# rom1504/clip-retrieval

Measured on AMD Instinct MI355X. Metric: images/sec embedded (ViT-L/14 bs=256; each sample = image + caption through both towers), higher is better.
Workload: dtype bf16

## Files before the change

### clip-retrieval_amd/csrc/clip_kernels.hip

```cpp

#include <hip/hip_runtime.h>
#include <stdint.h>
#include <stdlib.h>
#include <math.h>
#include "clip_kernels.h"
#include "gemm_common.h"
#include "clipx_attn_plan.h"

namespace clipx {

constexpr int G_TM = 128, G_TN = 128, G_BK = 64;
constexpr int G_STAGE_BYTES = (G_TM + G_TN) * G_BK * 2;
constexpr int G_GROUP_M = 8;

template <int EPI, bool GLDS, bool DEEP = false, bool F16 = false>
__global__ __launch_bounds__(256, (DEEP && !CLIPX_MFMA16) ? 1 : 2) void gemm_bf16_kernel(const bf16* __restrict__ A, const bf16* __restrict__ W,
                                                          const float* __restrict__ bias, void* __restrict__ outp,
                                                          const float* __restrict__ table, int T, int M, int N,
                                                          int K, int row0, const float* __restrict__ rowscale,
                                                          bf16* __restrict__ out16, int kz) {
  extern __shared__ __attribute__((aligned(16))) unsigned char smem[];
  const int tid = threadIdx.x;
  const int lane = tid & 63, w = tid >> 6;
  const int wn = w & 1, wm = w >> 1;
// ... 136 lines not shown
  D_DSREAD(Wd[sl][0], fW16[sl] + (so), 0);               \
  D_DSREAD(Wd[sl][1], fW16[sl] + (so), 2048);            \
  D_DSREAD(Wd[sl][2], fW16[sl] + (so), 4096);            \
  D_DSREAD(Wd[sl][3], fW16[sl] + (so), 6144);
#define D_READ_A(u, so)                                                \
  D_DSREAD(Ad[(u) & 1][0], fA16[(u) >> 1] + (so), ((u) & 1) * 2048);     \
  D_DSREAD(Ad[(u) & 1][1], fA16[(u) >> 1] + (so), 4096 + ((u) & 1) * 2048);
#define D_READ_U0(so) D_READ_W(0, so) D_READ_A(0, so) __builtin_amdgcn_sched_barrier(0);
#define D_READ_U1(so) D_READ_A(1, so) __builtin_amdgcn_sched_barrier(0);
#define D_READ_U2(so) D_READ_W(1, so) D_READ_A(2, so) __builtin_amdgcn_sched_barrier(0);
#define D_READ_U3(so) D_READ_A(3, so) __builtin_amdgcn_sched_barrier(0);
#define D_WAIT_N(n) asm volatile("s_waitcnt lgkmcnt(%0)" ::"n"(n) : "memory"); __builtin_amdgcn_sched_barrier(0);
#define D_MFMA_U(u)                                                                                                  \
  _Pragma("unroll") for (int i = 0; i < 2; ++i) _Pragma("unroll") for (int j = 0; j < 2; ++j)                        \
      _Pragma("unroll") for (int j2 = 0; j2 < 2; ++j2)                                                               \
          acc[i][j][2 * ((u) & 1) + j2] =                                                                            \
              mfma_16x16x32<F16>(Wd[(u) >> 1][2 * i + j2], Ad[(u) & 1][j], acc[i][j][2 * ((u) & 1) + j2]);           \
  __builtin_amdgcn_sched_barrier(0);
#else
#define D_READ(F, so, kk)                          \
  D_DSREAD(F[0], fW[kk] + (so), 0);                \
  D_DSREAD(F[1], fW[kk] + (so), 4096);             \
  D_DSREAD(F[2], fA[kk] + (so), 0);                \
  D_DSREAD(F[3], fA[kk] + (so), 4096);             \
  __builtin_amdgcn_sched_barrier(0);
#define D_WAIT_PREV() asm volatile("s_waitcnt lgkmcnt(4)" ::: "memory"); __builtin_amdgcn_sched_barrier(0);
#define D_MFMA(F)                                                                                                   \
  _Pragma("unroll") for (int i = 0; i < 2; ++i) _Pragma("unroll") for (int j = 0; j < 2; ++j) acc[i][j] =            \
      mfma_32x32x16<F16>(F[i], F[2 + j], acc[i][j]);                                                                   \
  __builtin_amdgcn_sched_barrier(0);
#endif
#define D_DMA(off, base, dst)                                                                                         \
  asm volatile("s_mov_b32 m0, %2\n\ts_nop 3\n\tglobal_load_lds_dwordx4 %0, %1" ::"v"(off), "s"(base), "s"(dst) : "memory")
      auto stage = [&](int t, int slot) {
        const char* bw = reinterpret_cast<const char*>(W) + (size_t)(t0 + t) * (G_BK * 2);
        const char* ba = reinterpret_cast<const char*>(A) + (size_t)(t0 + t) * (G_BK * 2);
        const unsigned d = lds_base + slot * G_STAGE_BYTES + wu * 4096;
#pragma unroll
        for (int i = 0; i < 4; ++i) {
          D_DMA(offW[i], bw, d + i * 1024);
          D_DMA(offA[i], ba, d + G_TN * G_BK * 2 + i * 1024);
        }
        __builtin_amdgcn_sched_barrier(0);
      };
      const int npro = nk < 4 ? nk : 4;
      for (int t = 0; t < npro; ++t) stage(t, t);
      if (npro == 4) asm volatile("s_waitcnt vmcnt(24)" ::: "memory");
      else if (npro == 3) asm volatile("s_waitcnt vmcnt(16)" ::: "memory");
      else if (npro == 2) asm volatile("s_waitcnt vmcnt(8)" ::: "memory");
      else asm volatile("s_waitcnt vmcnt(0)" ::: "memory");
      __builtin_amdgcn_sched_barrier(0);
      __builtin_amdgcn_s_barrier();
      __builtin_amdgcn_sched_barrier(0);
#if CLIPX_MFMA16
      D_READ_U0(0u)
      unsigned so = 0;
#define D_KT_HEAD()                                   \
  D_READ_U1(so) D_WAIT_N(2) D_MFMA_U(0)                \
  D_READ_U2(so) D_WAIT_N(6) D_MFMA_U(1)                \
  D_READ_U3(so) D_WAIT_N(2) D_MFMA_U(2)                \
  asm volatile("s_waitcnt lgkmcnt(0)" ::: "memory");  \
  __builtin_amdgcn_sched_barrier(0);
#define D_READ_FIRST(so_) D_READ_U0(so_)
#define D_MFMA_LAST() D_MFMA_U(3)
#else
      D_READ(F0, 0u, 0)
      unsigned so = 0;
#define D_KT_HEAD()                                   \
  D_READ(F1, so, 1) D_WAIT_PREV() D_MFMA(F0)           \
  D_READ(F0, so, 2) D_WAIT_PREV() D_MFMA(F1)           \
  D_READ(F1, so, 3) D_WAIT_PREV() D_MFMA(F0)           \
  asm volatile("s_waitcnt lgkmcnt(0)" ::: "memory");  \
  __builtin_amdgcn_sched_barrier(0);
#define D_READ_FIRST(so_) D_READ(F0, so_, 0)
#define D_MFMA_LAST() D_MFMA(F1)
#endif
#define D_SYNC(vm)                                           \
  asm volatile("s_waitcnt vmcnt(%0)" ::"i"(vm) : "memory");  \
  __builtin_amdgcn_sched_barrier(0);                         \
  __builtin_amdgcn_s_barrier();                              \
  __builtin_amdgcn_sched_barrier(0);
      int t = 0;
      for (; t + 4 < nk; ++t) {
        D_KT_HEAD()
        D_SYNC(16)
        stage(t + 4, t & 3);
        so = (so + G_STAGE_BYTES) & (4 * G_STAGE_BYTES - 1);
        D_READ_FIRST(so)
        D_MFMA_LAST()
      }
      for (; t < nk; ++t) {
        const int rem = nk - 1 - t;
        D_KT_HEAD()
        if (rem >= 3) { D_SYNC(16) } else if (rem == 2) { D_SYNC(8) } else { D_SYNC(0) }
        so = (so + G_STAGE_BYTES) & (4 * G_STAGE_BYTES - 1);
        if (rem > 0) { D_READ_FIRST(so) }
        D_MFMA_LAST()
      }
#undef D_DSREAD
#undef D_READ_FIRST
#undef D_MFMA_LAST
#undef D_DMA
#undef D_KT_HEAD
#undef D_SYNC
    } else {
    issue(0, 0);
    asm volatile("s_waitcnt vmcnt(0)" ::: "memory");
    __syncthreads();
    for (int t = 0; t < nk; ++t) {
      if (t + 1 < nk) issue(t + 1, (t + 1) & 1);
      compute(t & 1);
      asm volatile("s_waitcnt vmcnt(0)" ::: "memory");
      __syncthreads();
    }
    }
  } else {
    uint4 rw0, rw1, rw2, rw3, ra0, ra1, ra2, ra3;
#define G_LOAD(t)                                                             \
  {                                                                           \
    rw0 = *reinterpret_cast<const uint4*>(gW[0] + (size_t)(t) * G_BK);        \
    rw1 = *reinterpret_cast<const uint4*>(gW[1] + (size_t)(t) * G_BK);        \
    rw2 = *reinterpret_cast<const uint4*>(gW[2] + (size_t)(t) * G_BK);        \
    rw3 = *reinterpret_cast<const uint4*>(gW[3] + (size_t)(t) * G_BK);        \
    ra0 = *reinterpret_cast<const uint4*>(gA[0] + (size_t)(t) * G_BK);        \
    ra1 = *reinterpret_cast<const uint4*>(gA[1] + (size_t)(t) * G_BK);        \
    ra2 = *reinterpret_cast<const uint4*>(gA[2] + (size_t)(t) * G_BK);        \
    ra3 = *reinterpret_cast<const uint4*>(gA[3] + (size_t)(t) * G_BK);        \
  }
#define G_STORE(buf)                                                                        \
  {                                                                                         \
    unsigned char* dW = smem + (buf) * G_STAGE_BYTES + stage_off + lane * 16;               \
    *reinterpret_cast<uint4*>(dW) = rw0;                                                    \
    *reinterpret_cast<uint4*>(dW + 1024) = rw1;                                             \
    *reinterpret_cast<uint4*>(dW + 2048) = rw2;                                             \
    *reinterpret_cast<uint4*>(dW + 3072) = rw3;                                             \
    *reinterpret_cast<uint4*>(dW + G_TN * G_BK * 2) = ra0;                                  \
    *reinterpret_cast<uint4*>(dW + G_TN * G_BK * 2 + 1024) = ra1;                           \
    *reinterpret_cast<uint4*>(dW + G_TN * G_BK * 2 + 2048) = ra2;                           \
    *reinterpret_cast<uint4*>(dW + G_TN * G_BK * 2 + 3072) = ra3;                           \
  }
    G_LOAD(0)
    G_STORE(0)
    __syncthreads();
    for (int t = 0; t < nk; ++t) {
      if (t + 1 < nk) G_LOAD(t + 1)
      compute(t & 1);
      if (t + 1 < nk) G_STORE((t + 1) & 1)
      __syncthreads();
    }
#undef G_LOAD
#undef G_STORE
  }

#pragma unroll
  for (int j = 0; j < 2; ++j) {
#pragma unroll
    for (int i = 0; i < 2; ++i) {
#pragma unroll
      for (int g = 0; g < 4; ++g) {
        const int m = m0 + wm * 64 + j * 32 + quad_m(g, lane);
        if (m >= M) continue;
        const int n = n0 + wn * 64 + i * 32 + quad_n(g, lane);
        const float4 v = make_float4(G_ACC(i, j, g, 0), G_ACC(i, j, g, 1), G_ACC(i, j, g, 2), G_ACC(i, j, g, 3));
        gemm_store_quad<EPI>(v, m, n, N, bias, outp, table, T, row0, rowscale, out16);
      }
    }
  }
}

template <int EPI, bool F16 = false>
static hipError_t launch_gemm_epi(const GemmArgs& g, hipStream_t st) {
  const int ntm = (g.M + G_TM - 1) / G_TM, ntn = g.N / G_TN;
  const dim3 grid(ntm * ntn), block(256);
  const size_t smem = 2 * G_STAGE_BYTES;
  const bool small_off = (size_t)g.M * g.K * 2 < ((size_t)1 << 32) && (size_t)g.N * g.K * 2 < ((size_t)1 << 32);
  if (g.variant == 1 && g.K >= 2 * G_BK && small_off) {
    auto kern = gemm_bf16_kernel<EPI, true, true, F16>;
    const size_t smem4 = 4 * G_STAGE_BYTES;
    hipError_t e = hipFuncSetAttribute(reinterpret_cast<const void*>(kern), hipFuncAttributeMaxDynamicSharedMemorySize, (int)smem4);
    if (e != hipSuccess) return e;
    launch_with_events(g.events, kern, grid, block, smem4, st, g.A, g.W, g.bias, g.out, g.table, g.T, g.M, g.N, g.K, g.row0, g.rowscale, g.out16, 0);
  } else if (g.variant == 1) {
    auto kern = gemm_bf16_kernel<EPI, true, false, F16>;
    hipError_t e = hipFuncSetAttribute(reinterpret_cast<const void*>(kern), hipFuncAttributeMaxDynamicSharedMemorySize, (int)smem);
    if (e != hipSuccess) return e;
    launch_with_events(g.events, kern, grid, block, smem, st, g.A, g.W, g.bias, g.out, g.table, g.T, g.M, g.N, g.K, g.row0, g.rowscale, g.out16, 0);
  } else {
    auto kern = gemm_bf16_kernel<EPI, false, false, F16>;
    hipError_t e = hipFuncSetAttribute(reinterpret_cast<const void*>(kern), hipFuncAttributeMaxDynamicSharedMemorySize, (int)smem);
    if (e != hipSuccess) return e;
    launch_with_events(g.events, kern, grid, block, smem, st, g.A, g.W, g.bias, g.out, g.table, g.T, g.M, g.N, g.K, g.row0, g.rowscale, g.out16, 0);
  }
  return hipGetLastError();
}

template <int EPI>
__global__ __launch_bounds__(256) void splitk_reduce_kernel(const float* __restrict__ part, int S, int M, int N,
                                                           const float* __restrict__ bias, void* __restrict__ outp,
                                                           const float* __restrict__ rowscale, bf16* __restrict__ out16) {
  const int64_t q = (int64_t)blockIdx.x * 256 + threadIdx.x;
  const int nq4 = N >> 2;
  if (q >= (int64_t)M * nq4) return;
  const int m = (int)(q / nq4), n = (int)(q - (int64_t)m * nq4) * 4;
  float4 v = *reinterpret_cast<const float4*>(part + (size_t)m * N + n);
  for (int z = 1; z < S; ++z) {
    const float4 p = *reinterpret_cast<const float4*>(part + ((size_t)z * M + m) * N + n);
    v.x += p.x; v.y += p.y; v.z += p.z; v.w += p.w;
  }
  gemm_store_quad<EPI>(v, m, n, N, bias, outp, nullptr, 1, 0, rowscale, out16);
}

static int splitk_factor(const GemmArgs& g) {
  if (!g.splitk_ws || g.M > 1024 || g.epi == EPI_TABLE_F32 || g.epi == EPI_RAW_F32) return 1;
  const int nk = g.K / G_BK;
  if (nk < 8 || (nk < 32 && g.M > G_TM)) return 1;
  const int cu = g.n_cu > 0 ? g.n_cu : 256;
  const int tiles = ((g.M + G_TM - 1) / G_TM) * (g.N / G_TN);
  int S = 1;
  for (int c = 2; c <= 16; ++c) {
    if (nk % c != 0 || nk / c < 4) continue;
    if ((size_t)c * g.M * g.N * sizeof(float) > g.splitk_ws_bytes) break;
    if (tiles * (c - 1) >= cu) break;
    S = c;
  }
  return S;
}

template <int EPI>
static hipError_t launch_splitk_epi(const GemmArgs& g, int S, hipStream_t st) {
  const int ntm = (g.M + G_TM - 1) / G_TM, ntn = g.N / G_TN;
  auto kern = g.f16 ? gemm_bf16_kernel<EPI_RAW_F32, true, true, true> : gemm_bf16_kernel<EPI_RAW_F32, true, true, false>;
  const size_t smem4 = 4 * G_STAGE_BYTES;
  hipError_t e = hipFuncSetAttribute(reinterpret_cast<const void*>(kern), hipFuncAttributeMaxDynamicSharedMemorySize, (int)smem4);
  if (e != hipSuccess) return e;
  launch_with_events(g.events, kern, dim3(ntm * ntn, S), dim3(256), smem4, st, g.A, g.W, nullptr, g.splitk_ws, nullptr, 1, g.M, g.N, g.K, 0,
                     nullptr, nullptr, (g.K / G_BK) / S);
  const int64_t quads = (int64_t)g.M * (g.N / 4);
  launch_with_events(g.events, splitk_reduce_kernel<EPI>, dim3((unsigned)((quads + 255) / 256)), dim3(256), 0, st, g.splitk_ws, S, g.M, g.N,
                     g.bias, g.out, g.rowscale, g.out16);
  return hipGetLastError();
}

static hipError_t launch_gemm128(const GemmArgs& g, hipStream_t st) {
  const bool small_off = (size_t)g.M * g.K * 2 < ((size_t)1 << 32) && (size_t)g.N * g.K * 2 < ((size_t)1 << 32);
  const int S = (g.variant == 1 && small_off) ? splitk_factor(g) : 1;
  if (S > 1) {
    switch (g.epi) {
      case EPI_BIAS_BF16: return launch_splitk_epi<EPI_BIAS_BF16>(g, S, st);
      case EPI_BIAS_F16: return launch_splitk_epi<EPI_BIAS_F16>(g, S, st);
      case EPI_BIAS_QGELU_BF16: return launch_splitk_epi<EPI_BIAS_QGELU_BF16>(g, S, st);
      case EPI_BIAS_GELU_BF16: return launch_splitk_epi<EPI_BIAS_GELU_BF16>(g, S, st);
      case EPI_BIAS_RESID_F32: return launch_splitk_epi<EPI_BIAS_RESID_F32>(g, S, st);
      case EPI_BIAS_RESID_H16: return launch_splitk_epi<EPI_BIAS_RESID_H16>(g, S, st);
      default: break;
    }
  }
  if (g.f16) {
    switch (g.epi) {
      case EPI_BIAS_BF16: return launch_gemm_epi<EPI_BIAS_BF16, true>(g, st);
      case EPI_BIAS_F16: return launch_gemm_epi<EPI_BIAS_F16, true>(g, st);
      case EPI_BIAS_QGELU_BF16: return launch_gemm_epi<EPI_BIAS_QGELU_BF16, true>(g, st);
      case EPI_BIAS_GELU_BF16: return launch_gemm_epi<EPI_BIAS_GELU_BF16, true>(g, st);
      default: return hipErrorInvalidValue;
    }
  }
  switch (g.epi) {
    case EPI_BIAS_BF16: return launch_gemm_epi<EPI_BIAS_BF16>(g, st);
    case EPI_BIAS_F16: return launch_gemm_epi<EPI_BIAS_F16>(g, st);
    case EPI_BIAS_QGELU_BF16: return launch_gemm_epi<EPI_BIAS_QGELU_BF16>(g, st);
    case EPI_BIAS_GELU_BF16: return launch_gemm_epi<EPI_BIAS_GELU_BF16>(g, st);
    case EPI_BIAS_RESID_F32: return launch_gemm_epi<EPI_BIAS_RESID_F32>(g, st);
    case EPI_BIAS_RESID_H16: return launch_gemm_epi<EPI_BIAS_RESID_H16>(g, st);
    case EPI_TABLE_F32: return launch_gemm_epi<EPI_TABLE_F32>(g, st);
    default: return hipErrorInvalidValue;
  }
}

int gemm256_bulk_mtiles(int M, int N, int n_cu) {
  const int mt = M / 256, nt = N / 256;
  if (mt <= 0 || nt <= 0) return 0;
  const int cu = (n_cu > 0 ? n_cu : 256) & ~7;
  int best = mt;
  double best_cost = 1e30;
  for (int peel = 0; peel <= 8 && peel < mt; ++peel) {
    const int bulk = mt - peel;
    const int rounds = (bulk * nt + cu - 1) / cu;
    const double rest = (double)(peel * 4 * nt) / (2.0 * cu);
    const double cost = rounds + (peel ? 0.25 * (rest > 1.0 ? rest : 1.0) / 0.6 : 0.0);
    if (cost < best_cost - 1e-9) { best_cost = cost; best = bulk; }
  }
  return best;
}

int gemm256_tail_blocks(int N, int K, int n_cu) {
  int grid = (n_cu > 0 ? n_cu : 256) & ~7;
  if (grid < 8) grid = 8;
  if (N % 32 || K % 128 || (size_t)32 * K * 2 >= ((size_t)1 << 31)) return 0;
  const int cb = N / 32;
  for (int nb = 1; nb <= 4; ++nb)
    if (cb % nb == 0 && 8 * (cb / nb) <= grid) return nb;
  return 0;
}

int gemm256_dispatch_mtiles(int M, int N, int K, int variant, int n_cu) {
  if (variant < 2 || N % 256 != 0 || K % 128 != 0 || M < 256) return 0;
  const int bulk = gemm256_bulk_mtiles(M, N, n_cu);
  const int cu = (n_cu > 0 ? n_cu : 256);
  return bulk > 0 && (int64_t)bulk * (N / 256) >= cu / 2 ? bulk : 0;
}

int gemm256_whole_tile_rows(int M, int N, int K, int variant, int n_cu) {
  const int Mp = (M + 255) / 256 * 256;
  return Mp != M && gemm256_dispatch_mtiles(Mp, N, K, variant, n_cu) > 0 ? Mp : M;
}

hipError_t launch_gemm(const GemmArgs& g0, hipStream_t st) {
  GemmArgs g = g0;
  if (g.M <= 0 || g.N % G_TN != 0 || g.K % G_BK != 0 || g.K <= 0) return hipErrorInvalidValue;
  const bool out16 = g.epi == EPI_BIAS_BF16 || g.epi == EPI_BIAS_QGELU_BF16 || g.epi == EPI_BIAS_GELU_BF16 || g.epi == EPI_BIAS_F16;
  if (out16 && !g.rowscale) return hipErrorInvalidValue;
  if (g.f16 && !out16) return hipErrorInvalidValue;
  if (g.stats_eps > 0.f) {
    if (!g.f16 || !out16) return hipErrorInvalidValue;
    int fused_rows = 0;
    if (g.variant == 6 && g.N % 256 == 0 && g.K % 128 == 0 && g.M >= 256) {
      const int bulk = gemm256_bulk_mtiles(g.M, g.N, g.n_cu);
      const int cu = (g.n_cu > 0 ? g.n_cu : 256);
      GemmArgs b = g;
      b.M = bulk * 256;
      if (bulk > 0 && (int64_t)bulk * (g.N / 256) >= cu / 2 && gemm256w4_fuses_stats(b)) fused_rows = b.M;
    }
    if (fused_rows < g.M) {
      hipError_t e = launch_rowstats(reinterpret_cast<const char*>(g.A) + (size_t)fused_rows * g.K * 2, const_cast<float*>(g.rowscale) + fused_rows,
                                     g.M - fused_rows, g.K, g.stats_eps, st, 1, g.range_flag, 1, g.events);
      if (e != hipSuccess) return e;
    }
    if (fused_rows == 0) g.stats_eps = 0.f;
  }
  {
    const int bulk = gemm256_dispatch_mtiles(g.M, g.N, g.K, g.variant, g.n_cu);
    if (bulk > 0) {
      GemmArgs b = g;
      b.M = bulk * 256;
      b.tail_m0 = b.tail_nb = 0;
      if (g.M - b.M == 256 && (g.variant == 3 || g.variant == 6) && g.row0 == 0) {
        b.tail_nb = gemm256_tail_blocks(g.N, g.K, g.n_cu);
        b.tail_m0 = b.M;
      }
      const bool tail_inside = b.tail_nb > 0;
      hipError_t e = (g.variant == 6 && gemm256w4_supports(b)) ? launch_gemm256w4(b, g.n_cu, st) : launch_gemm256sp(b, g.n_cu, st);
      if (e != hipSuccess) return e;
      if (b.M == g.M || tail_inside) return hipSuccess;
      GemmArgs r = g;
      r.variant = 1;
      r.stats_eps = 0.f;
      r.splitk_ws = nullptr;
      r.A = g.A + (size_t)b.M * g.K;
      r.M = g.M - b.M;
      const size_t esz = (g.epi == EPI_BIAS_RESID_F32 || g.epi == EPI_TABLE_F32) ? 4 : 2;
      r.out = reinterpret_cast<char*>(g.out) + (size_t)b.M * g.N * esz;
      r.row0 = g.row0 + b.M;
      if (g.rowscale) r.rowscale = g.rowscale + b.M;
      if (g.out16) r.out16 = g.out16 + (size_t)b.M * g.N;
      return launch_gemm128(r, st);
    }
  }
  GemmArgs r = g;
  if (r.variant >= 2) r.variant = 1;
  r.stats_eps = 0.f;
  return launch_gemm128(r, st);
}

template <int NV, int OUT>
__global__ __launch_bounds__(256) void layernorm_kernel(const float* __restrict__ x, const float* __restrict__ gamma,
                                                       const float* __restrict__ beta, void* __restrict__ y, int M,
                                                       float eps, bf16* __restrict__ y16) {
  constexpr int d = NV * 256;
  const int lane = threadIdx.x & 63;
  const int row = blockIdx.x * 4 + (threadIdx.x >> 6);
  if (row >= M) return;
  const float4* xr = reinterpret_cast<const float4*>(x + (size_t)row * d);
  float4 v[NV];
  float s = 0.f;
#pragma unroll
  for (int e = 0; e < NV; ++e) {
    v[e] = xr[lane + 64 * e];
    s += (v[e].x + v[e].y) + (v[e].z + v[e].w);
  }
  for (int o = 32; o > 0; o >>= 1) s += __shfl_xor(s, o);
  const float mean = s * (1.f / d);
  float q = 0.f;
#pragma unroll
  for (int e = 0; e < NV; ++e) {
    const float a = v[e].x - mean, b = v[e].y - mean, c = v[e].z - mean, dd = v[e].w - mean;
    q += (a * a + b * b) + (c * c + dd * dd);
  }
  for (int o = 32; o > 0; o >>= 1) q += __shfl_xor(q, o);
  const float rstd = 1.f / sqrtf(q * (1.f / d) + eps);
#pragma unroll
  for (int e = 0; e < NV; ++e) {
    const int c4 = lane + 64 * e;
    const float4 g4 = reinterpret_cast<const float4*>(gamma)[c4];
    const float4 b4 = reinterpret_cast<const float4*>(beta)[c4];
    float4 o;
    o.x = (v[e].x - mean) * rstd * g4.x + b4.x;
    o.y = (v[e].y - mean) * rstd * g4.y + b4.y;
    o.z = (v[e].z - mean) * rstd * g4.z + b4.z;
    o.w = (v[e].w - mean) * rstd * g4.w + b4.w;
    if (OUT == 1) {
      bf16x4 ob;
      ob[0] = (bf16)o.x; ob[1] = (bf16)o.y; ob[2] = (bf16)o.z; ob[3] = (bf16)o.w;
      reinterpret_cast<bf16x4*>(reinterpret_cast<bf16*>(y) + (size_t)row * d)[c4] = ob;
    } else if (OUT == 2) {
      f16x4 oh;
      oh[0] = (_Float16)o.x; oh[1] = (_Float16)o.y; oh[2] = (_Float16)o.z; oh[3] = (_Float16)o.w;
      reinterpret_cast<f16x4*>(reinterpret_cast<_Float16*>(y) + (size_t)row * d)[c4] = oh;
    } else {
      reinterpret_cast<float4*>(reinterpret_cast<float*>(y) + (size_t)row * d)[c4] = o;
      if (y16) {
        bf16x4 ob;
        ob[0] = (bf16)o.x; ob[1] = (bf16)o.y; ob[2] = (bf16)o.z; ob[3] = (bf16)o.w;
        reinterpret_cast<bf16x4*>(y16 + (size_t)row * d)[c4] = ob;
      }
    }
  }
}

template <int NV2, bool F16>
__global__ __launch_bounds__(256) void rowstats_kernel(const void* __restrict__ x16, float* __restrict__ rstd, int M, float eps,
                                                       int* __restrict__ range_flag) {
  constexpr int d = NV2 * 256;
  const int lane = threadIdx.x & 63;
  const int row = blockIdx.x * 4 + (threadIdx.x >> 6);
  if (row >= M) return;
  const uint2* xr = reinterpret_cast<const uint2*>(reinterpret_cast<const uint16_t*>(x16) + (size_t)row * d);
  float v[NV2][4];
  float s = 0.f;
#pragma unroll
  for (int e = 0; e < NV2; ++e) {
    const uint2 raw = xr[lane + 64 * e];
    if (F16) {
      const f16x4 h = __builtin_bit_cast(f16x4, raw);
#pragma unroll
      for (int j = 0; j < 4; ++j) v[e][j] = (float)h[j];
    } else {
      const bf16x4 h = __builtin_bit_cast(bf16x4, raw);
#pragma unroll
      for (int j = 0; j < 4; ++j) v[e][j] = (float)h[j];
    }
    s += (v[e][0] + v[e][1]) + (v[e][2] + v[e][3]);
  }
  for (int o = 32; o > 0; o >>= 1) s += __shfl_xor(s, o);
  if (range_flag && lane == 0 && !(fabsf(s) <= 3.0e38f)) atomicOr(range_flag, 1);
  const float mean = s * (1.f / d);
  float q = 0.f;
#pragma unroll
  for (int e = 0; e < NV2; ++e) {
    const float a = v[e][0] - mean, b = v[e][1] - mean, c = v[e][2] - mean, dd = v[e][3] - mean;
    q += (a * a + b * b) + (c * c + dd * dd);
  }
  for (int o = 32; o > 0; o >>= 1) q += __shfl_xor(q, o);
  if (lane == 0) rstd[row] = 1.f / sqrtf(q * (1.f / d) + eps);
}

template <int NV2>
__global__ __launch_bounds__(256) void rowstats_f16_kernel(const void* __restrict__ x16, float* __restrict__ rstd, int M, float eps,
                                                           int* __restrict__ range_flag) {
  constexpr int d = NV2 * 256, NCH = d / 8;
  const int lane = threadIdx.x & 63, q4 = lane >> 4, r16 = lane & 15;
  const int row = (blockIdx.x * 4 + (threadIdx.x >> 6)) * 16 + r16;
  const uint4* xr = reinterpret_cast<const uint4*>(reinterpret_cast<const uint16_t*>(x16) + (size_t)(row < M ? row : M - 1) * d);
  const unsigned ones2 = __builtin_amdgcn_readfirstlane(0x3c003c00u);
  float s1 = 0.f, s2 = 0.f;
  constexpr int U = 8;
  static_assert((NCH / 4) % U == 0, "row length");
  for (int j0 = 0; j0 < NCH / 4; j0 += U) {
    uint4 c[U];
#pragma unroll
    for (int u = 0; u < U; ++u) c[u] = xr[q4 + 4 * (j0 + u)];
#pragma unroll
    for (int u = 0; u < U; ++u) {
      CLIPX_DOT2_SQ(s2, c[u].x); CLIPX_DOT2_SQ(s2, c[u].y); CLIPX_DOT2_SQ(s2, c[u].z); CLIPX_DOT2_SQ(s2, c[u].w);
      CLIPX_DOT2_SUM(s1, c[u].x, ones2); CLIPX_DOT2_SUM(s1, c[u].y, ones2); CLIPX_DOT2_SUM(s1, c[u].z, ones2); CLIPX_DOT2_SUM(s1, c[u].w, ones2);
    }
  }
  s1 += __shfl_xor(s1, 16);
  s2 += __shfl_xor(s2, 16);
  s1 += __shfl_xor(s1, 32);
  s2 += __shfl_xor(s2, 32);
  if (row >= M || q4 != 0) return;
  if (range_flag && !(fabsf(s1) <= 3.0e38f)) atomicOr(range_flag, 1);
  rstd[row] = ln_rstd_onepass(s1, s2, 1.f / (float)d, eps);
}

hipError_t launch_rowstats(const void* x16, float* rstd, int M, int d, float eps, hipStream_t st, int f16, int* range_flag, int canonical,
                           LaunchEvents* events) {
  if (M <= 0) return hipSuccess;
  if (f16 && canonical) {
    const dim3 grid((M + 63) / 64), block(256);
#define RSH_CASE(NV)                                                                                           \
  case NV * 256:                                                                                               \
    launch_with_events(events, rowstats_f16_kernel<NV>, grid, block, 0, st, x16, rstd, M, eps, range_flag);   \
    break;
    switch (d) {
      RSH_CASE(1) RSH_CASE(2) RSH_CASE(3) RSH_CASE(4) RSH_CASE(5) RSH_CASE(6) RSH_CASE(7) RSH_CASE(8)
      default: return hipErrorInvalidValue;
    }
#undef RSH_CASE
    return hipGetLastError();
  }
  const dim3 grid((M + 3) / 4), block(256);
#define RS_CASE(NV)                                                                                        \
  case NV * 256:                                                                                           \
    if (f16) launch_with_events(events, rowstats_kernel<NV, true>, grid, block, 0, st, x16, rstd, M, eps, range_flag);   \
    else launch_with_events(events, rowstats_kernel<NV, false>, grid, block, 0, st, x16, rstd, M, eps, range_flag);      \
    break;
  switch (d) {
    RS_CASE(1) RS_CASE(2) RS_CASE(3) RS_CASE(4) RS_CASE(5) RS_CASE(6) RS_CASE(7) RS_CASE(8)
    default: return hipErrorInvalidValue;
  }
#undef RS_CASE
  return hipGetLastError();
}

__global__ __launch_bounds__(256) void fold_layernorm_kernel(const float* __restrict__ W, const float* __restrict__ gamma,
                                                            const float* __restrict__ beta, const float* __restrict__ bias,
                                                            bf16* __restrict__ Wf, float* __restrict__ cf, int K, int f16) {
  __shared__ float red[8];
  const int n = blockIdx.x, tid = threadIdx.x;
  const float* w = W + (size_t)n * K;
  float sg = 0.f, sb = 0.f;
  for (int k = tid; k < K; k += 256) {
    sg += w[k] * gamma[k];
    sb += w[k] * beta[k];
  }
  for (int o = 32; o > 0; o >>= 1) { sg += __shfl_xor(sg, o); sb += __shfl_xor(sb, o); }
  if ((tid & 63) == 0) { red[tid >> 6] = sg; red[4 + (tid >> 6)] = sb; }
  __syncthreads();
  const float mean = (red[0] + red[1] + red[2] + red[3]) / (float)K;
  for (int k = tid; k < K; k += 256) {
    const float v = w[k] * gamma[k] - mean;
    if (f16) reinterpret_cast<_Float16*>(Wf)[(size_t)n * K + k] = (_Float16)v;
    else Wf[(size_t)n * K + k] = (bf16)v;
  }
  if (tid == 0) cf[n] = bias[n] + (red[4] + red[5] + red[6] + red[7]);
}
hipError_t launch_fold_layernorm(const float* W, const float* gamma, const float* beta, const float* bias, bf16* Wf, float* cf,
                                 int N, int K, hipStream_t st, int f16) {
  hipLaunchKernelGGL(fold_layernorm_kernel, dim3(N), dim3(256), 0, st, W, gamma, beta, bias, Wf, cf, K, f16);
  return hipGetLastError();
}
__global__ void fill_f32_kernel(float* __restrict__ p, float v, int64_t n) {
  for (int64_t i = (int64_t)blockIdx.x * blockDim.x + threadIdx.x; i < n; i += (int64_t)gridDim.x * blockDim.x) p[i] = v;
}
hipError_t launch_fill_f32(float* p, float v, int64_t n, hipStream_t st) {
  if (n <= 0) return hipSuccess;
  hipLaunchKernelGGL(fill_f32_kernel, dim3(256), dim3(256), 0, st, p, v, n);
  return hipGetLastError();
}

hipError_t launch_layernorm(const float* x, const float* gamma, const float* beta, void* y, int out_kind, int M, int d,
                            float eps, hipStream_t st, bf16* y16) {
  if (M <= 0) return hipSuccess;
  const dim3 grid((M + 3) / 4), block(256);
#define LN_CASE(NV)                                                                                           \
  case NV * 256:                                                                                              \
    if (out_kind == 1) hipLaunchKernelGGL((layernorm_kernel<NV, 1>), grid, block, 0, st, x, gamma, beta, y, M, eps, (bf16*)nullptr); \
    else if (out_kind == 2) hipLaunchKernelGGL((layernorm_kernel<NV, 2>), grid, block, 0, st, x, gamma, beta, y, M, eps, (bf16*)nullptr); \
    else hipLaunchKernelGGL((layernorm_kernel<NV, 0>), grid, block, 0, st, x, gamma, beta, y, M, eps, y16);    \
    break;
  switch (d) {
    LN_CASE(1) LN_CASE(2) LN_CASE(3) LN_CASE(4) LN_CASE(5) LN_CASE(6) LN_CASE(7) LN_CASE(8)
    default: return hipErrorInvalidValue;
  }
#undef LN_CASE
  return hipGetLastError();
}

template <int FMT>
__global__ __launch_bounds__(256) void im2col_kernel(const void* __restrict__ pixels, int B, int S, int P, int Kp,
                                                    float m0, float m1, float m2, float i0, float i1, float i2,
                                                    bf16* __restrict__ out) {
  const int gdim = S / P, T = gdim * gdim + 1, PP = P * P, K = 3 * PP, nch = Kp / 8;
  const int64_t total = (int64_t)B * T * nch;
  for (int64_t idx = (int64_t)blockIdx.x * blockDim.x + threadIdx.x; idx < total; idx += (int64_t)gridDim.x * blockDim.x) {
    const int ch = (int)(idx % nch);
    const int64_t row = idx / nch;
    const int t = (int)(row % T), b = (int)(row / T);
    bf16x8 o;
    const int tp = t > 0 ? t - 1 : 0;
    const int py = tp / gdim, px = tp - py * gdim;
    float raw[8];
    int cc[8];
#pragma unroll
    for (int e = 0; e < 8; ++e) {
      const int k = ch * 8 + e;
      const int kk = k < K ? k : K - 1;
      const int c = kk / PP, rem = kk - c * PP;
      const int iy = rem / P, ix = rem - iy * P;
      const int yy = py * P + iy, xx = px * P + ix;
      cc[e] = c;
      if (FMT == 0) raw[e] = reinterpret_cast<const float*>(pixels)[(((size_t)b * 3 + c) * S + yy) * S + xx];
      else raw[e] = (float)reinterpret_cast<const unsigned char*>(pixels)[(((size_t)b * S + yy) * S + xx) * 3 + c];
    }
#pragma unroll
    for (int e = 0; e < 8; ++e) {
      float v = raw[e];
      if (FMT != 0) {
        const int c = cc[e];
        const float mean = c == 0 ? m0 : (c == 1 ? m1 : m2), sd = c == 0 ? i0 : (c == 1 ? i1 : i2);
        v = __fdiv_rn(__fsub_rn(__fdiv_rn(v, 255.f), mean), sd);
      }
      o[e] = (t > 0 && ch * 8 + e < K) ? (bf16)v : (bf16)0.f;
    }
    *reinterpret_cast<bf16x8*>(out + (size_t)row * Kp + ch * 8) = o;
  }
}

hipError_t launch_im2col(const void* pixels, int fmt, int B, int S, int P, int Kp, const float* mean,
                         const float* stdv, bf16* out, hipStream_t st) {
  if (B <= 0) return hipSuccess;
  const int gdim = S / P, T = gdim * gdim + 1;
  const int64_t total = (int64_t)B * T * (Kp / 8);
  const int blocks = (int)((total + 255) / 256 < 65536 * 4 ? (total + 255) / 256 : 65536 * 4);
  if (fmt == 0)
    hipLaunchKernelGGL(im2col_kernel<0>, dim3(blocks), dim3(256), 0, st, pixels, B, S, P, Kp, 0.f, 0.f, 0.f, 1.f, 1.f, 1.f, out);
  else
    hipLaunchKernelGGL(im2col_kernel<1>, dim3(blocks), dim3(256), 0, st, pixels, B, S, P, Kp, mean[0], mean[1], mean[2],
                       stdv[0], stdv[1], stdv[2], out);
  return hipGetLastError();
}

__device__ __forceinline__ f32x16 attn_mfma(bf16x8 a, bf16x8 b, f32x16 c) {
  return __builtin_amdgcn_mfma_f32_32x32x16_f16(__builtin_bit_cast(f16x8, a), __builtin_bit_cast(f16x8, b), c, 0, 0, 0);
}
__device__ __forceinline__ unsigned attn_pack_p(float p0, float p1) {
  typedef float f32x2_t __attribute__((ext_vector_type(2)));
  typedef _Float16 f16x2_t __attribute__((ext_vector_type(2)));
  return __builtin_bit_cast(unsigned, __builtin_convertvector((f32x2_t){p0, p1}, f16x2_t));
}

__device__ long long g_attn_phase[8192 * 4];
#ifdef CLIPX_ABLATE
__device__ int g_attn_pk_timer = 0;
#endif
template <int DH, int NKB, int NW, int QPW, bool CAUSAL, bool RECOMP, bool TIMER = false, bool RAGGED = false>
__global__ __launch_bounds__(NW * 64, NKB > 9 ? (NW + 3) / 4 : (2 * NW + 3) / 4) void attention_kernel(const bf16* __restrict__ qkv, bf16* __restrict__ out, int Tin,
                                                              int H, float scale_log2e, int dbg, int q_blocks,
                                                              const int* __restrict__ offs, const int* __restrict__ lens) {
  constexpr int TP = NKB * 32;
  constexpr int CH = DH / 8;
  constexpr int KS = DH / 16;
  constexpr int KROW = DH == 64 ? 128 : 176;
  constexpr int DV = (DH + 31) / 32 * 32, NB = DV / 32;
  constexpr int VT_STRIDE = TP * 2 + 8;
  extern __shared__ __attribute__((aligned(16))) unsigned char smem[];
  unsigned char* sK = smem;
  unsigned char* sVt = smem + TP * KROW;
  const int tid = threadIdx.x, lane = tid & 63, w = tid >> 6;
  const int hb = lane >> 5, l31 = lane & 31;
  long long tph[4] = {0, 0, 0, 0};
  long long tst = TIMER ? (long long)__builtin_readcyclecounter() : 0;
#define A_STAMP(i) if (TIMER) { const long long n_ = (long long)__builtin_readcyclecounter(); tph[i] += n_ - tst; tst = n_; }
  const int b = blockIdx.x / H, h = blockIdx.x - b * H;
  const int ld = 3 * H * DH;
  const int T = lens ? lens[b] : Tin;
// ... 1335 lines not shown
```

### clip-retrieval_amd/csrc/gemm256_tail.h

```cpp
#pragma once
#include "gemm_common.h"

namespace clipx {

#ifndef S_FENCE
#define S_FENCE() __builtin_amdgcn_sched_barrier(0)
#endif

template <int EPI, bool F16, int NB, int NW = 8>
__device__ __forceinline__ void gemm256_tail(const bf16* __restrict__ A, const bf16* __restrict__ W, const float* __restrict__ bias,
                                             void* __restrict__ outp, const float* __restrict__ table, int T, int N, int K,
                                             const float* __restrict__ rowscale, bf16* __restrict__ out16, int tail_m0,
                                             unsigned char* smem, unsigned lds_base, int w, int lane) {
  constexpr int NOP = 1 + NB;
  constexpr int SB = NOP * 8192;
  constexpr int R = 131072 / SB;
  const int ncg = (N >> 5) / NB;
  const int strip = blockIdx.x;
  if (strip >= 8 * ncg) return;
  const int rb = strip & 7, cg = strip >> 3;
  const int tm = tail_m0 + rb * 32, tn = cg * NB * 32;
  const int l31 = lane & 31, hb = lane >> 5;
#if CLIPX_MFMA16
  const unsigned voff = (unsigned)(((lane & 15) * K + 8 * (lane >> 4)) * 2);
  const char* baseA = reinterpret_cast<const char*>(A) + (size_t)tm * K * 2;
  const char* baseW = reinterpret_cast<const char*>(W) + (size_t)tn * K * 2;
#define T_PIECE(p) ((size_t)(16 * ((p) & 1)) * K * 2 + ((p) >> 1) * 64)
  (void)l31; (void)hb;
#else
  const unsigned voff = (unsigned)((l31 * K + 8 * hb) * 2);
  const char* baseA = reinterpret_cast<const char*>(A) + (size_t)tm * K * 2;
  const char* baseW = reinterpret_cast<const char*>(W) + (size_t)tn * K * 2;
#define T_PIECE(p) ((size_t)(p) * 32)
#endif
  constexpr int PPW = 8 / NW;
  const int nch = K >> 7;
#define T_DMA(off, base, dst) \
  asm volatile("s_mov_b32 m0, %2\n\ts_nop 3\n\tglobal_load_lds_dwordx4 %0, %1" ::"v"(off), "s"(base), "s"(dst) : "memory")
  auto issue = [&](int c, int slot) {
    const int cc = c < nch ? c : nch - 1;
#pragma unroll
    for (int pp = 0; pp < PPW; ++pp) {
      const int p = w + NW * pp;
      const unsigned dst = lds_base + slot * SB + p * 1024;
      T_DMA(voff, baseA + T_PIECE(p) + (size_t)cc * 256, dst);
#pragma unroll
      for (int o = 0; o < NB; ++o) T_DMA(voff, baseW + T_PIECE(p) + (size_t)o * 64 * K + (size_t)cc * 256, dst + (1 + o) * 8192);
    }
    S_FENCE();
  };
#pragma unroll
  for (int c = 0; c < R - 1; ++c) issue(c, c);
#if CLIPX_MFMA16
  f32x4 acc[4];
#pragma unroll
  for (int g = 0; g < 4; ++g) acc[g] = f32x4{0.f, 0.f, 0.f, 0.f};
#define T_ACC(g, e) acc[g][e]
#else
  f32x16 acc;
#pragma unroll
  for (int r = 0; r < 16; ++r) acc[r] = 0.f;
#define T_ACC(g, e) acc[4 * (g) + (e)]
#endif
  int slot = 0;
  for (int c = 0; c < nch; ++c) {
    asm volatile("s_waitcnt vmcnt(%0)" ::"n"((R - 2) * NOP * PPW) : "memory");
    S_FENCE();
    __builtin_amdgcn_s_barrier();
    S_FENCE();
    issue(c + R - 1, slot == 0 ? R - 1 : slot - 1);
    if (w < NB) {
      const unsigned char* st = smem + slot * SB + lane * 16;
#if CLIPX_MFMA16
#pragma unroll
      for (int sl = 0; sl < 4; ++sl) {
        const frag_t af0 = *reinterpret_cast<const frag_t*>(st + (2 * sl) * 1024);
        const frag_t af1 = *reinterpret_cast<const frag_t*>(st + (2 * sl + 1) * 1024);
        const frag_t wf0 = *reinterpret_cast<const frag_t*>(st + (1 + w) * 8192 + (2 * sl) * 1024);
        const frag_t wf1 = *reinterpret_cast<const frag_t*>(st + (1 + w) * 8192 + (2 * sl + 1) * 1024);
        mfma_block16<F16>(acc, wf0, wf1, af0, af1);
      }
#else
#pragma unroll
      for (int ks = 0; ks < 8; ++ks) {
        const frag_t af = *reinterpret_cast<const frag_t*>(st + ks * 1024);
        const frag_t wf = *reinterpret_cast<const frag_t*>(st + (1 + w) * 8192 + ks * 1024);
        acc = mfma_32x32x16<F16>(wf, af, acc);
      }
#endif
    }
    slot = slot + 1 == R ? 0 : slot + 1;
  }
#undef T_DMA
#undef T_PIECE
  asm volatile("s_waitcnt vmcnt(0)" ::: "memory");
  S_FENCE();
  if (w < NB) {
#pragma unroll
    for (int g = 0; g < 4; ++g) {
      const int m = tm + quad_m(g, lane);
      const int n = tn + w * 32 + quad_n(g, lane);
      const float4 v = make_float4(T_ACC(g, 0), T_ACC(g, 1), T_ACC(g, 2), T_ACC(g, 3));
      gemm_store_quad<EPI>(v, m, n, N, bias, outp, table, T, 0, rowscale, out16);
    }
  }
#undef T_ACC
}


}
```

### clip-retrieval_amd/csrc/gemm_common.h

```cpp
#pragma once
#include <hip/hip_runtime.h>
#include <stdint.h>
#include "clip_kernels.h"

namespace clipx {

typedef __bf16 bf16x8 __attribute__((ext_vector_type(8)));
typedef __bf16 bf16x4 __attribute__((ext_vector_type(4)));
typedef float f32x16 __attribute__((ext_vector_type(16)));
typedef float f32x4 __attribute__((ext_vector_type(4)));
typedef _Float16 f16x8 __attribute__((ext_vector_type(8)));
typedef _Float16 f16x4 __attribute__((ext_vector_type(4)));
typedef int frag_t __attribute__((ext_vector_type(4)));

template <bool F16>
__device__ __forceinline__ f32x16 mfma_32x32x16(frag_t a, frag_t b, f32x16 c) {
  if constexpr (F16) return __builtin_amdgcn_mfma_f32_32x32x16_f16(__builtin_bit_cast(f16x8, a), __builtin_bit_cast(f16x8, b), c, 0, 0, 0);
  else return __builtin_amdgcn_mfma_f32_32x32x16_bf16(__builtin_bit_cast(bf16x8, a), __builtin_bit_cast(bf16x8, b), c, 0, 0, 0);
}
#ifndef CLIPX_MFMA16
#define CLIPX_MFMA16 1
#endif

template <bool F16>
__device__ __forceinline__ f32x4 mfma_16x16x32(frag_t a, frag_t b, f32x4 c) {
  if constexpr (F16) return __builtin_amdgcn_mfma_f32_16x16x32_f16(__builtin_bit_cast(f16x8, a), __builtin_bit_cast(f16x8, b), c, 0, 0, 0);
  else return __builtin_amdgcn_mfma_f32_16x16x32_bf16(__builtin_bit_cast(bf16x8, a), __builtin_bit_cast(bf16x8, b), c, 0, 0, 0);
}
template <bool F16>
__device__ __forceinline__ void mfma_block16(f32x4 (&q)[4], frag_t wf0, frag_t wf1, frag_t af0, frag_t af1) {
  q[0] = mfma_16x16x32<F16>(wf0, af0, q[0]);
  q[1] = mfma_16x16x32<F16>(wf1, af0, q[1]);
  q[2] = mfma_16x16x32<F16>(wf0, af1, q[2]);
  q[3] = mfma_16x16x32<F16>(wf1, af1, q[3]);
}
__device__ __forceinline__ int quad_m(int g, int lane) { return CLIPX_MFMA16 ? 16 * (g >> 1) + (lane & 15) : (lane & 31); }
__device__ __forceinline__ int quad_n(int g, int lane) { return CLIPX_MFMA16 ? 16 * (g & 1) + 4 * (lane >> 4) : 8 * g + 4 * (lane >> 5); }

__device__ __forceinline__ float ln_rstd_onepass(float s1, float s2, float inv_d, float eps) {
  const float mean = s1 * inv_d;
  const float ex2 = s2 * inv_d;
  float var = __builtin_fmaf(-mean, mean, ex2);
  var = var > 0.f ? var : 0.f;
  return 1.f / sqrtf(var + eps);
}
#define CLIPX_DOT2_SQ(acc, w) asm volatile("v_dot2_f32_f16 %0, %1, %1, %0" : "+v"(acc) : "v"(w))
#define CLIPX_DOT2_SUM(acc, w, ones) asm volatile("v_dot2_f32_f16 %0, %1, %2, %0" : "+v"(acc) : "v"(w), "s"(ones))

typedef __attribute__((address_space(3))) void* lds_ptr_t;
typedef const __attribute__((address_space(1))) void* gbl_ptr_t;

__device__ __forceinline__ float quick_gelu(float v) {
  return v * __builtin_amdgcn_rcpf(1.f + __builtin_amdgcn_exp2f(-1.702f * 1.4426950408889634f * v));
}
__device__ __forceinline__ float gelu_erf(float v) {
  const float z = fabsf(v) * 0.70710678118654752f;
  const float t = __builtin_amdgcn_rcpf(__builtin_fmaf(0.3275911f, z, 1.f));
  float p = __builtin_fmaf(1.061405429f, t, -1.453152027f);
  p = __builtin_fmaf(p, t, 1.421413741f);
  p = __builtin_fmaf(p, t, -0.284496736f);
  p = __builtin_fmaf(p, t, 0.254829592f);
  const float e = __builtin_amdgcn_exp2f(-1.4426950408889634f * z * z);
  const float erf_abs = __builtin_fmaf(-p * t, e, 1.f);
  return 0.5f * v + 0.5f * fabsf(v) * erf_abs;
}

template <int EPI>
__device__ __forceinline__ void gemm_store_quad(float4 v, int m, int n, int N, const float* __restrict__ bias,
                                                void* __restrict__ outp, const float* __restrict__ table, int T,
                                                int row0, const float* __restrict__ rowscale, bf16* __restrict__ out16) {
  constexpr bool OUT_BF16 = EPI == EPI_BIAS_BF16 || EPI == EPI_BIAS_QGELU_BF16 || EPI == EPI_BIAS_GELU_BF16 || EPI == EPI_BIAS_F16;
  if (EPI == EPI_RAW_F32) {
    *reinterpret_cast<float4*>(reinterpret_cast<float*>(outp) + (size_t)m * N + n) = v;
    return;
  }
  if (EPI != EPI_TABLE_F32) {
    const float4 b4 = *reinterpret_cast<const float4*>(bias + n);
    if (OUT_BF16) {
      const float r = rowscale[m];
      v.x = __builtin_fmaf(v.x, r, b4.x); v.y = __builtin_fmaf(v.y, r, b4.y);
      v.z = __builtin_fmaf(v.z, r, b4.z); v.w = __builtin_fmaf(v.w, r, b4.w);
    } else {
      v.x += b4.x; v.y += b4.y; v.z += b4.z; v.w += b4.w;
    }
  }
  if (EPI == EPI_BIAS_QGELU_BF16) { v.x = quick_gelu(v.x); v.y = quick_gelu(v.y); v.z = quick_gelu(v.z); v.w = quick_gelu(v.w); }
  if (EPI == EPI_BIAS_GELU_BF16) { v.x = gelu_erf(v.x); v.y = gelu_erf(v.y); v.z = gelu_erf(v.z); v.w = gelu_erf(v.w); }
  if (EPI == EPI_BIAS_F16) {
    asm volatile("" : "+v"(v.x), "+v"(v.y), "+v"(v.z), "+v"(v.w));
    f16x4 o;
    o[0] = (_Float16)v.x; o[1] = (_Float16)v.y; o[2] = (_Float16)v.z; o[3] = (_Float16)v.w;
    *reinterpret_cast<f16x4*>(reinterpret_cast<_Float16*>(outp) + (size_t)m * N + n) = o;
  } else if (OUT_BF16) {
    bf16x4 o;
    o[0] = (bf16)v.x; o[1] = (bf16)v.y; o[2] = (bf16)v.z; o[3] = (bf16)v.w;
    *reinterpret_cast<bf16x4*>(reinterpret_cast<bf16*>(outp) + (size_t)m * N + n) = o;
  } else if (EPI == EPI_BIAS_RESID_F32) {
    float4* p = reinterpret_cast<float4*>(reinterpret_cast<float*>(outp) + (size_t)m * N + n);
    float4 o = *p;
    o.x += v.x; o.y += v.y; o.z += v.z; o.w += v.w;
    *p = o;
    if (out16) {
      bf16x4 h;
      h[0] = (bf16)o.x; h[1] = (bf16)o.y; h[2] = (bf16)o.z; h[3] = (bf16)o.w;
      *reinterpret_cast<bf16x4*>(out16 + (size_t)m * N + n) = h;
    }
  } else if (EPI == EPI_BIAS_RESID_H16) {
    f16x4* p = reinterpret_cast<f16x4*>(reinterpret_cast<_Float16*>(outp) + (size_t)m * N + n);
    const f16x4 x4 = *p;
    f16x4 h;
    h[0] = (_Float16)((float)x4[0] + v.x); h[1] = (_Float16)((float)x4[1] + v.y);
    h[2] = (_Float16)((float)x4[2] + v.z); h[3] = (_Float16)((float)x4[3] + v.w);
    *p = h;
  } else {
    const float4 t4 = *reinterpret_cast<const float4*>(table + (size_t)((m + row0) % T) * N + n);
    v.x += t4.x; v.y += t4.y; v.z += t4.z; v.w += t4.w;
    *reinterpret_cast<float4*>(reinterpret_cast<float*>(outp) + (size_t)m * N + n) = v;
  }
}

hipError_t launch_gemm256sp(const GemmArgs& g, int n_cu, hipStream_t st);
bool gemm256w4_supports(const GemmArgs& g);
bool gemm256w4_fuses_stats(const GemmArgs& g);
hipError_t launch_gemm256w4(const GemmArgs& g, int n_cu, hipStream_t st);

}
```

Measured before the change: 6072.

## Add standalone strip GEMM kernel for small-M and tail rows with swizzled LDS

Adds a standalone strip kernel, reusing the fused tail routine, that handles GEMMs with M≤256 and leftover 256-row tails. Before this, those went to the generic 128-tile kernel. The tail routine gets an XOR-swizzled LDS layout for the MFMA16 path and a 'deal' mode that spreads the MFMA quads over all 4 waves instead of idling the extra waves. It also gates fusing the tail into the bulk kernel on whether the bulk tile count is large enough to hide it. This targets poor occupancy and wave imbalance on small GEMMs such as text-tower or tail launches, at the risk of layout bugs and extra launches.

After: 6125, median of 6. About the same (+0.9%).

```diff
diff --git a/clip-retrieval_amd/csrc/clip_kernels.hip b/clip-retrieval_amd/csrc/clip_kernels.hip
--- a/clip-retrieval_amd/csrc/clip_kernels.hip
+++ b/clip-retrieval_amd/csrc/clip_kernels.hip
@@ -462,11 +462,30 @@
   return 0;
 }
 
+static int gemm256_min_tiles(int n_cu) {
+  const int cu = (n_cu > 0 ? n_cu : 256);
+#ifdef CLIPX_ABLATE
+  if (const char* mt = getenv("CLIPX_GEMM_MIN_TILES")) return atoi(mt);
+#endif
+  return cu / 2;
+}
+
 int gemm256_dispatch_mtiles(int M, int N, int K, int variant, int n_cu) {
   if (variant < 2 || N % 256 != 0 || K % 128 != 0 || M < 256) return 0;
   const int bulk = gemm256_bulk_mtiles(M, N, n_cu);
-  const int cu = (n_cu > 0 ? n_cu : 256);
-  return bulk > 0 && (int64_t)bulk * (N / 256) >= cu / 2 ? bulk : 0;
+  return bulk > 0 && (int64_t)bulk * (N / 256) >= gemm256_min_tiles(n_cu) ? bulk : 0;
+}
+
+static bool gemm256_tail_rides(int64_t ntiles, int N, int nb, int n_cu) {
+  int grid = (n_cu > 0 ? n_cu : 256) & ~7;
+  if (grid < 8) grid = 8;
+  const int cpx = grid >> 3, ncg = (N / 32) / nb;
+  return ntiles >= 7 * cpx + ncg;
+}
+
+static int gemm256_strip_width(const GemmArgs& g) {
+  if ((g.variant != 3 && g.variant != 6) || g.splitk_ws || !gemm256_strips_supports(g)) return 0;
+  return gemm256_tail_blocks(g.N, g.K, g.n_cu);
 }
 
 int gemm256_whole_tile_rows(int M, int N, int K, int variant, int n_cu) {
@@ -488,7 +507,7 @@
       const int cu = (g.n_cu > 0 ? g.n_cu : 256);
       GemmArgs b = g;
       b.M = bulk * 256;
-      if (bulk > 0 && (int64_t)bulk * (g.N / 256) >= cu / 2 && gemm256w4_fuses_stats(b)) fused_rows = b.M;
+      if (bulk > 0 && (int64_t)bulk * (g.N / 256) >= gemm256_min_tiles(cu) && gemm256w4_fuses_stats(b)) fused_rows = b.M;
     }
     if (fused_rows < g.M) {
       hipError_t e = launch_rowstats(reinterpret_cast<const char*>(g.A) + (size_t)fused_rows * g.K * 2, const_cast<float*>(g.rowscale) + fused_rows,
@@ -496,6 +515,10 @@
       if (e != hipSuccess) return e;
     }
     if (fused_rows == 0) g.stats_eps = 0.f;
+  }
+  if (g.M <= 256) {
+    const int nb = gemm256_strip_width(g);
+    if (nb > 0) return launch_gemm256_strips(g, nb, st);
   }
   {
     const int bulk = gemm256_dispatch_mtiles(g.M, g.N, g.K, g.variant, g.n_cu);
@@ -504,24 +527,31 @@
       b.M = bulk * 256;
       b.tail_m0 = b.tail_nb = 0;
       if (g.M - b.M == 256 && (g.variant == 3 || g.variant == 6) && g.row0 == 0) {
-        b.tail_nb = gemm256_tail_blocks(g.N, g.K, g.n_cu);
-        b.tail_m0 = b.M;
+        const int nb = gemm256_tail_blocks(g.N, g.K, g.n_cu);
+        if (nb > 0 && gemm256_tail_rides((int64_t)bulk * (g.N / 256), g.N, nb, g.n_cu)) {
+          b.tail_nb = nb;
+          b.tail_m0 = b.M;
+        }
       }
       const bool tail_inside = b.tail_nb > 0;
       hipError_t e = (g.variant == 6 && gemm256w4_supports(b)) ? launch_gemm256w4(b, g.n_cu, st) : launch_gemm256sp(b, g.n_cu, st);
       if (e != hipSuccess) return e;
       if (b.M == g.M || tail_inside) return hipSuccess;
       GemmArgs r = g;
-      r.variant = 1;
       r.stats_eps = 0.f;
       r.splitk_ws = nullptr;
       r.A = g.A + (size_t)b.M * g.K;
       r.M = g.M - b.M;
       const size_t esz = (g.epi == EPI_BIAS_RESID_F32 || g.epi == EPI_TABLE_F32) ? 4 : 2;
       r.out = reinterpret_cast<char*>(g.out) + (size_t)b.M * g.N * esz;
-      r.row0 = g.row0 + b.M;
       if (g.rowscale) r.rowscale = g.rowscale + b.M;
       if (g.out16) r.out16 = g.out16 + (size_t)b.M * g.N;
+      if (r.M == 256 && g.row0 == 0) {
+        const int nb = gemm256_strip_width(r);
+        if (nb > 0) return launch_gemm256_strips(r, nb, st);
+      }
+      r.variant = 1;
+      r.row0 = g.row0 + b.M;
       return launch_gemm128(r, st);
     }
   }
diff --git a/clip-retrieval_amd/csrc/gemm256_strips.hip b/clip-retrieval_amd/csrc/gemm256_strips.hip
--- /dev/null
+++ b/clip-retrieval_amd/csrc/gemm256_strips.hip
@@ -0,0 +1,71 @@
+
+#include <hip/hip_runtime.h>
+#include <stdint.h>
+#include "gemm_common.h"
+#include "gemm256_tail.h"
+
+namespace clipx {
+
+constexpr int STRIPS_LDS = 131072;
+
+template <int EPI, bool F16, int NB>
+__global__ __launch_bounds__(256) void gemm256_strips_kernel(const bf16* __restrict__ A, const bf16* __restrict__ W, const float* __restrict__ bias,
+                                                             void* __restrict__ outp, int N, int K, const float* __restrict__ rowscale, int nrb) {
+  extern __shared__ __attribute__((aligned(16))) unsigned char smem[];
+  const int lane = threadIdx.x & 63;
+  const int w = __builtin_amdgcn_readfirstlane(threadIdx.x >> 6);
+  const unsigned lds_base = __builtin_amdgcn_readfirstlane((unsigned)(uintptr_t)(__attribute__((address_space(3))) unsigned char*)smem);
+  const int strip = ((int)blockIdx.x / nrb) * 8 + (int)blockIdx.x % nrb;
+  gemm256_tail_strip<EPI, F16, NB, 4>(A, W, bias, outp, nullptr, 1, N, K, rowscale, nullptr, 0, smem, lds_base, w, lane, strip);
+}
+
+template <int EPI, bool F16, int NB>
+static hipError_t launch_strips_nb(const GemmArgs& g, hipStream_t st) {
+  auto kern = gemm256_strips_kernel<EPI, F16, NB>;
+  hipError_t e = hipFuncSetAttribute(reinterpret_cast<const void*>(kern), hipFuncAttributeMaxDynamicSharedMemorySize, STRIPS_LDS);
+  if (e != hipSuccess) return e;
+  const int nrb = g.M / 32, ncg = (g.N / 32) / NB;
+  launch_with_events(g.events, kern, dim3(nrb * ncg), dim3(256), (size_t)STRIPS_LDS, st, g.A, g.W, g.bias, g.out, g.N, g.K, g.rowscale, nrb);
+  return hipGetLastError();
+}
+
+template <int EPI, bool F16>
+static hipError_t launch_strips_epi(const GemmArgs& g, int nb, hipStream_t st) {
+  switch (nb) {
+    case 1: return launch_strips_nb<EPI, F16, 1>(g, st);
+    case 2: return launch_strips_nb<EPI, F16, 2>(g, st);
+    case 3: return launch_strips_nb<EPI, F16, 3>(g, st);
+    case 4: return launch_strips_nb<EPI, F16, 4>(g, st);
+    default: return hipErrorInvalidValue;
+  }
+}
+
+bool gemm256_strips_supports(const GemmArgs& g) {
+  if (g.M <= 0 || g.M > 256 || g.M % 32 != 0 || g.N % 32 != 0 || g.K % 128 != 0 || g.row0 != 0) return false;
+  const bool out16 = g.epi == EPI_BIAS_BF16 || g.epi == EPI_BIAS_F16 || g.epi == EPI_BIAS_QGELU_BF16 || g.epi == EPI_BIAS_GELU_BF16;
+  if (out16) return g.rowscale != nullptr;
+  return !g.f16 && g.epi == EPI_BIAS_RESID_H16;
+}
+
+hipError_t launch_gemm256_strips(const GemmArgs& g, int nb, hipStream_t st) {
+  if (!gemm256_strips_supports(g) || nb < 1 || nb > 4 || (g.N / 32) % nb != 0) return hipErrorInvalidValue;
+  if (g.f16) {
+    switch (g.epi) {
+      case EPI_BIAS_BF16: return launch_strips_epi<EPI_BIAS_BF16, true>(g, nb, st);
+      case EPI_BIAS_F16: return launch_strips_epi<EPI_BIAS_F16, true>(g, nb, st);
+      case EPI_BIAS_QGELU_BF16: return launch_strips_epi<EPI_BIAS_QGELU_BF16, true>(g, nb, st);
+      case EPI_BIAS_GELU_BF16: return launch_strips_epi<EPI_BIAS_GELU_BF16, true>(g, nb, st);
+      default: return hipErrorInvalidValue;
+    }
+  }
+  switch (g.epi) {
+    case EPI_BIAS_BF16: return launch_strips_epi<EPI_BIAS_BF16, false>(g, nb, st);
+    case EPI_BIAS_F16: return launch_strips_epi<EPI_BIAS_F16, false>(g, nb, st);
+    case EPI_BIAS_QGELU_BF16: return launch_strips_epi<EPI_BIAS_QGELU_BF16, false>(g, nb, st);
+    case EPI_BIAS_GELU_BF16: return launch_strips_epi<EPI_BIAS_GELU_BF16, false>(g, nb, st);
+    case EPI_BIAS_RESID_H16: return launch_strips_epi<EPI_BIAS_RESID_H16, false>(g, nb, st);
+    default: return hipErrorInvalidValue;
+  }
+}
+
+}
diff --git a/clip-retrieval_amd/csrc/gemm256_tail.h b/clip-retrieval_amd/csrc/gemm256_tail.h
--- a/clip-retrieval_amd/csrc/gemm256_tail.h
+++ b/clip-retrieval_amd/csrc/gemm256_tail.h
@@ -8,24 +8,30 @@
 #endif
 
 template <int EPI, bool F16, int NB, int NW = 8>
-__device__ __forceinline__ void gemm256_tail(const bf16* __restrict__ A, const bf16* __restrict__ W, const float* __restrict__ bias,
-                                             void* __restrict__ outp, const float* __restrict__ table, int T, int N, int K,
-                                             const float* __restrict__ rowscale, bf16* __restrict__ out16, int tail_m0,
-                                             unsigned char* smem, unsigned lds_base, int w, int lane) {
+__device__ __forceinline__ void gemm256_tail_strip(const bf16* __restrict__ A, const bf16* __restrict__ W, const float* __restrict__ bias,
+                                                   void* __restrict__ outp, const float* __restrict__ table, int T, int N, int K,
+                                                   const float* __restrict__ rowscale, bf16* __restrict__ out16, int tail_m0,
+                                                   unsigned char* smem, unsigned lds_base, int w, int lane, int strip) {
   constexpr int NOP = 1 + NB;
   constexpr int SB = NOP * 8192;
   constexpr int R = 131072 / SB;
+  constexpr bool DEAL = CLIPX_MFMA16 && NW == 4 && NB < 4;
   const int ncg = (N >> 5) / NB;
-  const int strip = blockIdx.x;
   if (strip >= 8 * ncg) return;
   const int rb = strip & 7, cg = strip >> 3;
   const int tm = tail_m0 + rb * 32, tn = cg * NB * 32;
   const int l31 = lane & 31, hb = lane >> 5;
 #if CLIPX_MFMA16
-  const unsigned voff = (unsigned)(((lane & 15) * K + 8 * (lane >> 4)) * 2);
+  const int prow = (w & 3) * 8 + (lane >> 3);
+  const unsigned voff = (unsigned)((prow * K + (((lane & 7) ^ ((prow >> 1) & 7)) << 3)) * 2);
   const char* baseA = reinterpret_cast<const char*>(A) + (size_t)tm * K * 2;
   const char* baseW = reinterpret_cast<const char*>(W) + (size_t)tn * K * 2;
-#define T_PIECE(p) ((size_t)(16 * ((p) & 1)) * K * 2 + ((p) >> 1) * 64)
+#define T_PIECE(p) ((size_t)(((p) >> 2) * 128))
+  unsigned fo[2];
+#pragma unroll
+  for (int s2 = 0; s2 < 2; ++s2) fo[s2] = (unsigned)((lane & 15) * 128 + (((4 * s2 + (lane >> 4)) ^ (((lane & 15) >> 1) & 7)) << 4));
+#define T_SLAB(sl) (fo[(sl) & 1] + ((sl) >> 1) * 4096)
+  constexpr unsigned HALF_B = 2048;
   (void)l31; (void)hb;
 #else
   const unsigned voff = (unsigned)((l31 * K + 8 * hb) * 2);
@@ -56,6 +62,13 @@
 #pragma unroll
   for (int g = 0; g < 4; ++g) acc[g] = f32x4{0.f, 0.f, 0.f, 0.f};
 #define T_ACC(g, e) acc[g][e]
+  unsigned qa[NB], qw[NB];
+#pragma unroll
+  for (int i = 0; i < NB; ++i) {
+    const int q = NB * w + i;
+    qa[i] = (unsigned)(((q & 3) >> 1) * HALF_B);
+    qw[i] = (unsigned)((1 + (q >> 2)) * 8192 + (q & 1) * HALF_B);
+  }
 #else
   f32x16 acc;
 #pragma unroll
@@ -69,22 +82,35 @@
     __builtin_amdgcn_s_barrier();
     S_FENCE();
     issue(c + R - 1, slot == 0 ? R - 1 : slot - 1);
-    if (w < NB) {
-      const unsigned char* st = smem + slot * SB + lane * 16;
+    if (DEAL) {
+#if CLIPX_MFMA16
+      const unsigned char* st = smem + slot * SB;
+#pragma unroll
+      for (int sl = 0; sl < 4; ++sl) {
+#pragma unroll
+        for (int i = 0; i < NB; ++i) {
+          const frag_t af = *reinterpret_cast<const frag_t*>(st + qa[i] + T_SLAB(sl));
+          const frag_t wf = *reinterpret_cast<const frag_t*>(st + qw[i] + T_SLAB(sl));
+          acc[i] = mfma_16x16x32<F16>(wf, af, acc[i]);
+        }
+      }
+#endif
+    } else if (w < NB) {
+      const unsigned char* st = smem + slot * SB;
 #if CLIPX_MFMA16
 #pragma unroll
       for (int sl = 0; sl < 4; ++sl) {
-        const frag_t af0 = *reinterpret_cast<const frag_t*>(st + (2 * sl) * 1024);
-        const frag_t af1 = *reinterpret_cast<const frag_t*>(st + (2 * sl + 1) * 1024);
-        const frag_t wf0 = *reinterpret_cast<const frag_t*>(st + (1 + w) * 8192 + (2 * sl) * 1024);
-        const frag_t wf1 = *reinterpret_cast<const frag_t*>(st + (1 + w) * 8192 + (2 * sl + 1) * 1024);
+        const frag_t af0 = *reinterpret_cast<const frag_t*>(st + T_SLAB(sl));
+        const frag_t af1 = *reinterpret_cast<const frag_t*>(st + T_SLAB(sl) + HALF_B);
+        const frag_t wf0 = *reinterpret_cast<const frag_t*>(st + (1 + w) * 8192 + T_SLAB(sl));
+        const frag_t wf1 = *reinterpret_cast<const frag_t*>(st + (1 + w) * 8192 + T_SLAB(sl) + HALF_B);
         mfma_block16<F16>(acc, wf0, wf1, af0, af1);
       }
 #else
 #pragma unroll
       for (int ks = 0; ks < 8; ++ks) {
-        const frag_t af = *reinterpret_cast<const frag_t*>(st + ks * 1024);
-        const frag_t wf = *reinterpret_cast<const frag_t*>(st + (1 + w) * 8192 + ks * 1024);
+        const frag_t af = *reinterpret_cast<const frag_t*>(st + lane * 16 + ks * 1024);
+        const frag_t wf = *reinterpret_cast<const frag_t*>(st + lane * 16 + (1 + w) * 8192 + ks * 1024);
         acc = mfma_32x32x16<F16>(wf, af, acc);
       }
 #endif
@@ -93,9 +119,21 @@
   }
 #undef T_DMA
 #undef T_PIECE
+#if CLIPX_MFMA16
+#undef T_SLAB
+#endif
   asm volatile("s_waitcnt vmcnt(0)" ::: "memory");
   S_FENCE();
-  if (w < NB) {
+  if (DEAL) {
+#pragma unroll
+    for (int i = 0; i < NB; ++i) {
+      const int q = NB * w + i, o = q >> 2, g = q & 3;
+      const int m = tm + quad_m(g, lane);
+      const int n = tn + o * 32 + quad_n(g, lane);
+      const float4 v = make_float4(T_ACC(i, 0), T_ACC(i, 1), T_ACC(i, 2), T_ACC(i, 3));
+      gemm_store_quad<EPI>(v, m, n, N, bias, outp, table, T, 0, rowscale, out16);
+    }
+  } else if (w < NB) {
 #pragma unroll
     for (int g = 0; g < 4; ++g) {
       const int m = tm + quad_m(g, lane);
@@ -107,5 +145,12 @@
 #undef T_ACC
 }
 
+template <int EPI, bool F16, int NB, int NW = 8>
+__device__ __forceinline__ void gemm256_tail(const bf16* __restrict__ A, const bf16* __restrict__ W, const float* __restrict__ bias,
+                                             void* __restrict__ outp, const float* __restrict__ table, int T, int N, int K,
+                                             const float* __restrict__ rowscale, bf16* __restrict__ out16, int tail_m0,
+                                             unsigned char* smem, unsigned lds_base, int w, int lane) {
+  gemm256_tail_strip<EPI, F16, NB, NW>(A, W, bias, outp, table, T, N, K, rowscale, out16, tail_m0, smem, lds_base, w, lane, (int)blockIdx.x);
+}
 
 }
diff --git a/clip-retrieval_amd/csrc/gemm_common.h b/clip-retrieval_amd/csrc/gemm_common.h
--- a/clip-retrieval_amd/csrc/gemm_common.h
+++ b/clip-retrieval_amd/csrc/gemm_common.h
@@ -123,5 +123,7 @@
 bool gemm256w4_supports(const GemmArgs& g);
 bool gemm256w4_fuses_stats(const GemmArgs& g);
 hipError_t launch_gemm256w4(const GemmArgs& g, int n_cu, hipStream_t st);
+bool gemm256_strips_supports(const GemmArgs& g);
+hipError_t launch_gemm256_strips(const GemmArgs& g, int nb, hipStream_t st);
 
 }
```
